# sideprotocol/plonky2-gpu

Hardware: AMD Instinct MI355X
Metric: NTTs/sec at 2^20 Goldilocks (higher is better)
Workload: dtype u64 (Goldilocks, integer modular)

## Files before the change

plonky2_gpu_amd/csrc/poseidon.h:

```cpp
#pragma once
#include "poseidon_vector.h"

namespace poseidon {

using poseidon_vector::HALF_FULL;
using poseidon_vector::N_PARTIAL;
using poseidon_vector::W;

typedef int v4i32 __attribute__((ext_vector_type(4)));
typedef int v16i32 __attribute__((ext_vector_type(16)));

#ifdef POSEIDON_MDS_NATURAL
#include POSEIDON_MDS_NATURAL
#else
struct MdsOperands {
    v4i32 A;
    v16i32 C;
};

__device__ __forceinline__ uint32_t mds_row_word(uint32_t o) {
    constexpr uint32_t WORDS[12] = POSEIDON_MDS_ROW_WORDS;
    uint32_t x = 0;
#pragma unroll
    for (int k = 0; k < 12; k++) x = o == (uint32_t)k ? WORDS[k] : x;
    return x;
}

__device__ __forceinline__ MdsOperands mds_operands() {
    const uint32_t lane = __builtin_amdgcn_mbcnt_hi(~0u, __builtin_amdgcn_mbcnt_lo(~0u, 0u));
    const uint32_t m = lane & 31, h = lane >> 5;
    const uint32_t r = (m & 3) + 4 * (m >> 3);
    const bool on = ((m >> 2) & 1) == h && r < 12;
    MdsOperands o;
#pragma unroll
    for (int w = 0; w < 3; w++) o.A[w] = on ? (int)mds_row_word((4 * w + 12 - r) % 12) : 0;
    o.A[3] = 0;
#pragma unroll
    for (int k = 0; k < 16; k++) o.C[k] = POSEIDON_MDS_PLANE_OFFSET;
    asm volatile("" : "+v"(o.A), "+v"(o.C));
    return o;
}

__device__ __forceinline__ void require_full_wave() {
    if (__builtin_amdgcn_read_exec() != ~0ull) __builtin_trap();
}

#ifdef POSEIDON_MDS_LAYER
#include POSEIDON_MDS_LAYER
#else
__device__ __forceinline__ void mds_layer(uint64_t (&s)[W], const MdsOperands &ops, const uint32_t *__restrict__ xy) {
    v4i32 T[8];
#pragma unroll
    for (int G = 0; G < 3; G++)
#pragma unroll
        for (int h = 0; h < 2; h++) {
            const uint32_t r0 = (uint32_t)(s[4 * G] >> (32 * h)), r1 = (uint32_t)(s[4 * G + 1] >> (32 * h));
            const uint32_t r2 = (uint32_t)(s[4 * G + 2] >> (32 * h)), r3 = (uint32_t)(s[4 * G + 3] >> (32 * h));
            const uint32_t a01 = __builtin_amdgcn_perm(r1, r0, 0x05010400u), c01 = __builtin_amdgcn_perm(r1, r0, 0x07030602u);
            const uint32_t a23 = __builtin_amdgcn_perm(r3, r2, 0x05010400u), c23 = __builtin_amdgcn_perm(r3, r2, 0x07030602u);
            T[4 * h + 0][G] = (int)(__builtin_amdgcn_perm(a23, a01, 0x05040100u) ^ 0x80808080u);
            T[4 * h + 1][G] = (int)(__builtin_amdgcn_perm(a23, a01, 0x07060302u) ^ 0x80808080u);
            T[4 * h + 2][G] = (int)(__builtin_amdgcn_perm(c23, c01, 0x05040100u) ^ 0x80808080u);
            T[4 * h + 3][G] = (int)(__builtin_amdgcn_perm(c23, c01, 0x07060302u) ^ 0x80808080u);
        }
    const uint32_t x0l = (uint32_t)s[0], x0h = (uint32_t)(s[0] >> 32);
    uint64_t al[W], ah[W];
    {
        const v16i32 D0 = __builtin_amdgcn_mfma_i32_32x32x32_i8(ops.A, T[0], ops.C, 0, 0, 0), D2 = __builtin_amdgcn_mfma_i32_32x32x32_i8(ops.A, T[2], ops.C, 0, 0, 0);
        const v16i32 D1 = __builtin_amdgcn_mfma_i32_32x32x32_i8(ops.A, T[1], ops.C, 0, 0, 0), D3 = __builtin_amdgcn_mfma_i32_32x32x32_i8(ops.A, T[3], ops.C, 0, 0, 0);
#pragma unroll
        for (int r = 0; r < W; r++) {
            const uint32_t Al = (uint32_t)D0[r] | ((uint32_t)D2[r] << 16), Bl = (uint32_t)D1[r] | ((uint32_t)D3[r] << 16);
            al[r] = ((uint64_t)xy[2 * r] << 32) | Al;
            asm("v_mad_u64_u32 %0, vcc, %1, %2, %0" : "+v"(al[r]) : "v"(Bl), "s"(256u) : "vcc");
        }
    }
    {
        const v16i32 D4 = __builtin_amdgcn_mfma_i32_32x32x32_i8(ops.A, T[4], ops.C, 0, 0, 0), D6 = __builtin_amdgcn_mfma_i32_32x32x32_i8(ops.A, T[6], ops.C, 0, 0, 0);
        const v16i32 D5 = __builtin_amdgcn_mfma_i32_32x32x32_i8(ops.A, T[5], ops.C, 0, 0, 0), D7 = __builtin_amdgcn_mfma_i32_32x32x32_i8(ops.A, T[7], ops.C, 0, 0, 0);
#pragma unroll
        for (int r = 0; r < W; r++) {
            const uint32_t Ah = (uint32_t)D4[r] | ((uint32_t)D6[r] << 16), Bh = (uint32_t)D5[r] | ((uint32_t)D7[r] << 16);
            ah[r] = ((uint64_t)xy[2 * r + 1] << 32) | Ah;
            asm("v_mad_u64_u32 %0, vcc, %1, %2, %0" : "+v"(ah[r]) : "v"(Bh), "s"(256u) : "vcc");
        }
    }
    asm("v_mad_u64_u32 %0, vcc, %2, %4, %0\n\t"
        "v_mad_u64_u32 %1, vcc, %3, %4, %1"
        : "+v"(al[0]), "+v"(ah[0])
        : "v"(x0l), "v"(x0h), "n"(POSEIDON_MDS_DIAG0)
        : "vcc");
#pragma unroll
    for (int r = 0; r < W; r++) s[r] = gl::fold96(al[r], ah[r]);
}

#endif
#endif

__device__ __forceinline__ void full_round(uint64_t (&s)[W], const MdsOperands &ops, const uint32_t *__restrict__ xy) {
#pragma unroll
    for (int i = 0; i < W; i++) s[i] = gl::pow7(s[i]);
    mds_layer(s, ops, xy);
}

__device__ __forceinline__ void permute(uint64_t (&s)[W], const MdsOperands &ops) {
    require_full_wave();
#pragma unroll
    for (int i = 0; i < W; i++) s[i] = gl::add_canonical(s[i], POSEIDON_ALL_ROUND_CONSTANTS[i]);
#pragma unroll 1
    for (int r = 0; r < HALF_FULL; r++) full_round(s, ops, POSEIDON_MDS_XY + 2 * W * r);
#pragma unroll 1
    for (int r = HALF_FULL; r < HALF_FULL + N_PARTIAL; r++) {
        s[0] = gl::pow7(s[0]);
        mds_layer(s, ops, POSEIDON_MDS_XY + 2 * W * r);
    }
#pragma unroll 1
    for (int r = HALF_FULL + N_PARTIAL; r < 2 * HALF_FULL + N_PARTIAL; r++) full_round(s, ops, POSEIDON_MDS_XY + 2 * W * r);
}

}
```

plonky2_gpu_amd/csrc/poseidon_limb_constants.h:

```cpp
#pragma once
#include <stdint.h>
#ifndef POSEIDON_CONST
#define POSEIDON_CONST static const
#endif
#define POSEIDON_PARTIAL_BLOCK_TERMS 297

POSEIDON_CONST uint64_t POSEIDON_INIT_STREAM_C0[121] __attribute__((aligned(64))) = {
    0x80772dc2645b280bULL, 0xe796d293a47a64cbULL, 0xdcedab70f40718baULL, 0xf4a437f2888ae909ULL,
    0xf97abba0dffb6c50ULL, 0x7f8e41e0b0a6cdffULL, 0x726af914971c1374ULL, 0x64dd936da878404dULL,
    0x85418a9fef8a9890ULL, 0x156048ee7a738154ULL, 0xd841e8ef9dde8ba0ULL, 0xdc927721da922cf8ULL,
    0xb124c33152a2421aULL, 0x14a4a64da0b2668fULL, 0xc537d44dc2875403ULL, 0x5e40f0c9bb82aab5ULL,
    0x4b1ba8d40afca97dULL, 0x1d7f8a2cce1a9d00ULL, 0x4db9a2ead2bd7262ULL, 0xd8a2eb7ef5e707adULL,
    0x91f7562377e81df5ULL, 0x156048ee7a738154ULL, 0xc1978156516879adULL, 0x0ee5dc0ce131268aULL,
    0x4715b8e5ab34653bULL, 0x7f68007619fd8ba9ULL, 0x5996a80497e24a6bULL, 0x623708f28fca70e8ULL,
    0x18737784700c75cdULL, 0xbe2e19f6d07f1a83ULL, 0xbfe85ababed2d882ULL, 0xd8a2eb7ef5e707adULL,
    0x85418a9fef8a9890ULL, 0x90e80c591f48b603ULL, 0xa9032a52f930fae6ULL, 0x1e8916a99c93a88eULL,
    0xa4911db6a32612daULL, 0x07084430a7307c9aULL, 0xbf150dc4914d380fULL, 0x7fb45d605dd82838ULL,
    0x02290fe23c20351aULL, 0xbe2e19f6d07f1a83ULL, 0x4db9a2ead2bd7262ULL, 0x64dd936da878404dULL,
    0x3a2432625475e3aeULL, 0x7e33ca8c814280deULL, 0xbba4b5d86b9a3b2cULL, 0x2f7e9aade3fdaec1ULL,
    0xad2f570a5b8545aaULL, 0xc26a083554767106ULL, 0x862361aeab0f9b6eULL, 0x7fb45d605dd82838ULL,
    0x18737784700c75cdULL, 0x1d7f8a2cce1a9d00ULL, 0x726af914971c1374ULL, 0x00a2d4321cca94feULL,
    0xad11180f69a8c29eULL, 0xe76649f9bd5d5c2eULL, 0xe7ffd578da4ea43dULL, 0xab7f81fef4274770ULL,
    0x753b8b1126665c22ULL, 0xc26a083554767106ULL, 0xbf150dc4914d380fULL, 0x623708f28fca70e8ULL,
    0x4b1ba8d40afca97dULL, 0x7f8e41e0b0a6cdffULL, 0x77736f524010c932ULL, 0xc75ac6d5b5a10ff3ULL,
// ... 478 lines not shown
    0x4cdb240000000000ULL, 0x004e640000000000ULL, 0xc0539dd594c2eb25ULL, 0x53a4361a08c316b6ULL,
    0xb8899f8b277ef3a5ULL, 0xdd56375f98e8540aULL, 0x20d61b073e4d24ccULL, 0x0eaa137ccdfcaeedULL,
    0x4bd5386cb93533f0ULL, 0xa92f07522603d627ULL, 0x79442e109481d1b7ULL, 0x90bb65609b16866aULL,
    0x14ac4d5b709acc24ULL, 0x6188d0c1cbd8533eULL, 0xb110adc5ffc6f63aULL, 0x50ae6232ffffc1cdULL,
    0x9f6aa442ffffffbdULL, 0x4cdb240000000000ULL, 0x004e640000000000ULL, 0xc8c9a691f64cf04aULL,
    0x4ee06eac4803f9d2ULL, 0xef75547931cea75cULL, 0x509c4977f0df603dULL, 0x6bcad519b6a4680dULL,
    0x96ac65b9ee5f7156ULL, 0xfe3d76217a264e25ULL, 0x27e0c04ae42f912dULL, 0x76c119b2058a2a42ULL,
    0xbfc4898b7337bacfULL, 0x7d6abe160558056aULL, 0xce2601ac466ca224ULL, 0x6188d0c1cbd8533eULL,
    0xb110adc5ffc6f63aULL, 0x50ae6232ffffc1cdULL, 0x9f6aa442ffffffbdULL, 0x4cdb240000000000ULL,
    0x004e640000000000ULL, 0x4fbdff13b945cae5ULL, 0x36077a68e217ddc4ULL, 0xa16b9056ee536ff4ULL,
    0x6f90ce44d6523d8fULL, 0x4545ea2780307b14ULL, 0xde188deac917d1a0ULL, 0x2f6cd10ea2c7415aULL,
    0x0032d62b81ce4f49ULL, 0x68e53b0c643d5a60ULL, 0x1f565def76440b0eULL, 0xcd963151269f4c14ULL,
    0xaee48b63151f6cf1ULL, 0xce2601ac466ca224ULL, 0x6188d0c1cbd8533eULL, 0xb110adc5ffc6f63aULL,
    0x50ae6232ffffc1cdULL, 0x9f6aa442ffffffbdULL, 0x4cdb240000000000ULL, 0x004e640000000000ULL,
    0xc3e553c640e2f627ULL, 0x6129993ec2f23203ULL, 0xc8c12f675f4a311fULL, 0x2e9055ab3feb7226ULL,
    0xaa2f94298328fa67ULL, 0x3aa2cd0e195d72d5ULL, 0xeb96c11d2ba82d97ULL, 0xd2eaf60942c686c8ULL,
    0x0a0781d3857dbb7aULL, 0x4bff0687c17fb73cULL, 0x20829e1121be8986ULL, 0x09eff43fc38db9cdULL,
    0xaee48b63151f6cf1ULL, 0xce2601ac466ca224ULL, 0x6188d0c1cbd8533eULL, 0xb110adc5ffc6f63aULL,
    0x50ae6232ffffc1cdULL, 0x9f6aa442ffffffbdULL, 0x4cdb240000000000ULL, 0x004e640000000000ULL,
    0x82124bbd051fc758ULL, 0x182c413a98d88851ULL, 0x703aca58966b498aULL, 0x5d40546d4259451cULL,
    0x85efc9ddc2389549ULL, 0x683141d10a2580ecULL, 0x7f14503670bb9c01ULL, 0x3423c537de869e0aULL,
    0x11dfc42b97c160faULL, 0xe2b5aa9a9ed4d540ULL, 0x180bfc04feba6fccULL, 0x93e511ff2f214401ULL,
    0x09eff43fc38db9cdULL, 0xaee48b63151f6cf1ULL, 0xce2601ac466ca224ULL, 0x6188d0c1cbd8533eULL,
    0xb110adc5ffc6f63aULL, 0x50ae6232ffffc1cdULL, 0x9f6aa442ffffffbdULL, 0x4cdb240000000000ULL,
    0x004e640000000000ULL, 0x3c72d754b84cea98ULL, 0x72fd1e97d56494daULL, 0xfdd528147a800c90ULL,
    0x69f4ae409e14b190ULL, 0x31bbb09fcc35af60ULL, 0x6ba3f325ffc76cdaULL, 0x5ef29dc4ffffc23bULL,
    0x4c5ce043ffffffbcULL, 0x47dc600000000000ULL, 0x004c000000000000ULL, 0x0000500000000000ULL,
    0xf6754bac41d188f1ULL, 0xc9e9e8c22168e4f9ULL, 0x06eb78e061df7f6eULL, 0xda550f299e7a10abULL,
    0x5721ef3cd09930c3ULL, 0xb562ee26ffcc31d9ULL, 0x1b6558bfffffc740ULL, 0x5b56203cffffffc3ULL,
    0x42db200000000000ULL, 0x005d400000000000ULL, 0x0000880000000000ULL, 0x4ea6bd499ea511e9ULL,
    0x9e5bc61b931f9ec5ULL, 0xc167f24a3b9a79c7ULL, 0x7b4e75e7fd4b21e8ULL, 0x3c63baa9cb88dd56ULL,
    0xfddef831ffc69fceULL, 0x6047d698ffffc167ULL, 0x143e1843ffffffbcULL, 0x4d2a580000000000ULL,
    0x0045380000000000ULL, 0x0000480000000000ULL, 0xcb5c52d5a439fe0dULL, 0xbf73379506c3ebe5ULL,
    0xa340b60b8b47de82ULL, 0xdd379ecee40e9d06ULL, 0x3d720756d0e1b4a9ULL, 0x5fb4b57effcc8681ULL,
    0x49f8f433ffffc7ccULL, 0x123d3c3dffffffc2ULL, 0x433dfc0000000000ULL, 0x004c7c0000000000ULL,
    0x00009c0000000000ULL, 0xea231a946ac6c26aULL, 0x8fb9fe055fac72cfULL, 0x61a2e9179c4336ceULL,
    0x64286e4accdd5d85ULL, 0xce3ccec7cb547d38ULL, 0x01405989ffc67276ULL, 0x2ff98b05ffffc0faULL,
    0x549f4c43ffffffbcULL, 0x49340c0000000000ULL, 0x0059ec0000000000ULL, 0x0000340000000000ULL,
    0x23bfe07c96e52509ULL, 0x675cd2dd5b461196ULL, 0x218e7dd3c14759c7ULL, 0xe31bb6c37bd4cd0cULL,
    0x4760004acafb03b5ULL, 0xa2077e05ffc605faULL, 0x0b64433fffffc0c0ULL, 0x0da68444ffffffbbULL,
    0x4fe2840000000000ULL, 0x004dc40000000000ULL, 0x0000340000000000ULL, 0xf47208ed0dd292bfULL,
    0x7c0de42d324421e4ULL, 0x08b3e1b289905464ULL, 0xe8b496ec3273c8e6ULL, 0x2d68aa33cdefb5ccULL,
    0x3ded0f9dffc95062ULL, 0x91879bb4ffffc44bULL, 0xbcbce040ffffffbfULL, 0x45f1600000000000ULL,
    0x0048c00000000000ULL, 0x0000700000000000ULL, 0xf20c883ffd83c064ULL, 0xd3633a161f2810f8ULL,
    0xe741c972500558a2ULL, 0x24bb9832d06db79bULL, 0x75daff51c92850aeULL, 0x2b513c52ffc413adULL,
    0x589d91a0ffffbe5fULL, 0x8b2a5046ffffffb9ULL, 0x4cb2500000000000ULL, 0x0060b00000000000ULL,
    0x0000080000000000ULL, 0x28b6e2a7c4612060ULL, 0xbcf8538e4c81c079ULL, 0x711cb1f50b1d6224ULL,
    0xf278288605e2174aULL, 0xeb9c1cc8cb922337ULL, 0xd12595d0ffc6aa2fULL, 0x8dbd7e7fffffc180ULL,
    0x28a7c043ffffffbcULL, 0x4d3f000000000000ULL, 0x004da00000000000ULL, 0x0000400000000000ULL,
    0x5b9d8087c5ddd8dbULL, 0x6b71eb5c31ba931dULL, 0xe799d7986ab1847eULL, 0xd5f75a6b61bea969ULL,
    0x80fcb72fd053ccd0ULL, 0x7d3f19c1ffcbea3eULL, 0xc4fbbceaffffc715ULL, 0xa7d7043dffffffc2ULL,
    0x4282440000000000ULL, 0x003cc40000000000ULL, 0x0000a40000000000ULL, 0x550810f4d60c836bULL,
    0x41065b24228d5d31ULL, 0x7f0db99480d05ea8ULL, 0x2f6f8fe32bc933edULL, 0xe08adac7cbbc6938ULL,
    0x25e4de42ffc6e5bdULL, 0x83db8290ffffc16fULL, 0xd8974442ffffffbdULL, 0x4a25840000000000ULL,
    0x0057240000000000ULL, 0x00003c0000000000ULL,
};

#define POSEIDON_MDS_ROW_WORDS {0x10290f11u, 0x0210290fu, 0x1c021029u, 0x0d1c0210u, 0x0d0d1c02u, 0x270d0d1cu, 0x12270d0du, 0x2212270du, 0x14221227u, 0x11142212u, 0x0f111422u, 0x290f1114u}
#define POSEIDON_MDS_PLANE_OFFSET 32768
#define POSEIDON_MDS_DIAG0 8

POSEIDON_CONST uint32_t POSEIDON_MDS_XY[720] __attribute__((aligned(64))) = {
    0x7d4b40a3u, 0x08dd377fu, 0x9b8ea8e0u, 0xbe3e71aau, 0x0d16df22u, 0xb6a23a8cu, 0x93eecc47u, 0x1095f87fu,
    0x0cdfd3f0u, 0x23abe934u, 0xfd7b015eu, 0x70cf3f63u, 0xa7be7ab2u, 0xf2707305u, 0x91a93619u, 0x51b790c8u,
    0x958db98bu, 0x4039b805u, 0xdc62ad13u, 0xe6fc00f4u, 0x1b38723eu, 0x6963b419u, 0xc922e83au, 0xf7344452u,
    0x0bd863cdu, 0xde21ff7eu, 0x8b09cd56u, 0x6a659ff3u, 0xfe10254eu, 0xf9c6ee9au, 0xb51970dbu, 0xcd7da250u,
    0x9073326bu, 0x1cf4d376u, 0xa94a2d54u, 0x0307aca2u, 0x68ed8564u, 0xe73d5278u, 0x68ac854eu, 0xeef4cfbeu,
    0xd39cb892u, 0x931f1a7cu, 0x6640103eu, 0xa7629bb1u, 0xcb7634b1u, 0x24eaf29fu, 0x127b826eu, 0x163d69cdu,
    0x10d2eafau, 0x81d46bedu, 0x6fd0a772u, 0x01169a7au, 0xb1204affu, 0x507d13e3u, 0xe1b5922au, 0x8db99cadu,
    0x64d56371u, 0x181eb35fu, 0xe883b5b5u, 0x795b9bc6u, 0x97b3c511u, 0xee28848au, 0x0556a27cu, 0x463ef8cdu,
    0x90c27cb5u, 0x57fbc1a9u, 0xdc9b42b7u, 0x19257967u, 0x4aa0a17fu, 0xf6108b40u, 0x7161df70u, 0x34d529cfu,
    0x5511ec9bu, 0xe7b20bf7u, 0x8606cf7du, 0xa840ce44u, 0x156d214eu, 0x59dcbcbau, 0xff74753au, 0x21c87284u,
    0xb8521bb8u, 0xa2b2157cu, 0xa6231c1au, 0xfcbb295eu, 0xbb7f9e02u, 0xb5840cf7u, 0xea4e8f0fu, 0x68d86cfeu,
    0x95d0fe97u, 0x13fdb8b9u, 0xe31a9e2cu, 0x44de4e5cu, 0x1ad8586eu, 0xe212f76du, 0x416b1589u, 0xb95be98bu,
    0x97bf27d2u, 0xd9728273u, 0x28b41300u, 0x6a9cf061u, 0x5d15c720u, 0x503d9405u, 0xdf663a85u, 0x66c1bb41u,
    0x1d4ec3edu, 0x470e33a8u, 0x2f128705u, 0xf509e9e8u, 0x1131e668u, 0x9b86fa0fu, 0x83873129u, 0xb3b0b8b2u,
    0xcf4a5deau, 0x18a0004au, 0x5a9ea6dau, 0x36403dc6u, 0x3d728a8au, 0x943f636eu, 0xb1ab0e1eu, 0x59ba39fdu,
    0xa1c142e7u, 0xf7ebd7c4u, 0x17a146dfu, 0x2be935b3u, 0x7bf858d9u, 0x3a158ae4u, 0xb90c0427u, 0x1090a744u,
    0x10d4d292u, 0x58d11b01u, 0x7d4fe00eu, 0xe12b528eu, 0x5fd4f48eu, 0xffebb77au, 0x6c52d15du, 0xc688b135u,
    0x630f5cadu, 0xa7cf0cefu, 0x8d06b75du, 0xefbea0deu, 0x67467522u, 0x1e9929b1u, 0x54379c01u, 0x11cd434fu,
    0xc5dbe551u, 0x25a910b8u, 0x9e6ee872u, 0x3bf19fc3u, 0x0ff9efc4u, 0x7f9e0e7du, 0x4032c3e6u, 0x690c8477u,
    0xf61dbe52u, 0x70e72a9cu, 0xeceb0ac6u, 0xe1f8dee6u, 0x33c17f27u, 0x1d4b8f3fu, 0x61c27839u, 0x946fc710u,
    0x0af65bceu, 0x005a3111u, 0xd73cad47u, 0x1b04c343u, 0xf1b8b359u, 0x6f2ea8cfu, 0x9c827028u, 0x099f0d64u,
    0x3505debfu, 0x3c53ee72u, 0x338623d0u, 0x50152ac0u, 0x8fd1493bu, 0x7d6df523u, 0x6e653f66u, 0x21184458u,
    0x62163f4au, 0x15f8e2fau, 0xdf6f6e7au, 0x0c21e9ccu, 0xf8550594u, 0xd9490c79u, 0x7fced201u, 0x81a01339u,
    0x4493b9c6u, 0x86cc1b89u, 0x26b58618u, 0x8602bb61u, 0x8419603eu, 0x1808b8ceu, 0x0123723du, 0x5c45c9dfu,
    0x9fa5a65fu, 0x3d496139u, 0x17e60d77u, 0x257d84edu, 0xfe3cce7fu, 0xe4372f18u, 0x6eb18146u, 0xd2dd812au,
    0x41290130u, 0x4afcfc74u, 0xdb83adcau, 0x51373f83u, 0x2d2fc472u, 0x3229223eu, 0x86615f67u, 0xa1e4f145u,
    0x4b750e34u, 0x17e6254bu, 0x748cd80eu, 0x2b0d2b61u, 0x679a3d1bu, 0x51a3e8f2u, 0x2a85a256u, 0x86224893u,
    0x5d1c83c9u, 0x7359a8f4u, 0x47773baeu, 0xed4fb40au, 0x3ad3cbc8u, 0x05eb3eeeu, 0x330cb1d0u, 0x83a8bf2du,
    0x880aed55u, 0xd21ccbabu, 0x68786438u, 0x492d4d2eu, 0x70f49ecfu, 0x162e41deu, 0xf6e564afu, 0x81a97f04u,
    0x29f908ebu, 0xeaae1d7bu, 0x37ab1b49u, 0x610c4be7u, 0x2746bcb2u, 0x944cf1c6u, 0x8c7e3355u, 0x9c7f07afu,
    0xc3c9eb8du, 0x6cda7c78u, 0x953b5ceeu, 0x9e42631eu, 0x9d91a162u, 0x385b00e3u, 0xdc34dd40u, 0x9b2d8642u,
    0xa0d40c26u, 0x21102899u, 0x5652213du, 0xac4713ddu, 0x5ff97265u, 0x52dae480u, 0xe33bbc09u, 0x5b6315f4u,
    0xcdc36804u, 0x5baf4127u, 0x9c0601b6u, 0x841b6c21u, 0xd6448796u, 0xd7bb6139u, 0x68758d60u, 0xb3d82dbcu,
    0x98c43ee3u, 0x7cdd2ba7u, 0xb863b895u, 0x802659f6u, 0xddeed6d2u, 0x45120f04u, 0x7744fb8bu, 0xb81eaefbu,
    0x60922f52u, 0x91313d97u, 0x3f5181efu, 0xe7c68f36u, 0x5660ac01u, 0x8f235693u, 0x508d8bf1u, 0xfd0e304du,
    0x5360b322u, 0x96d50908u, 0x039d5c83u, 0x1544bec9u, 0x43f0f4bbu, 0xda4aab0bu, 0x8f4e6c60u, 0x9687d702u,
    0x1f79b1f7u, 0x3ac569bbu, 0x457a8f71u, 0x960472c8u, 0xc636e856u, 0xee2b1e03u, 0x8d3fcb15u, 0xbc827fcfu,
    0xe8be8b93u, 0xeed4fa99u, 0x1deaa0f2u, 0x8cf27015u, 0x5bec4377u, 0x684f2a98u, 0x71772164u, 0x7119035eu,
    0x94094edcu, 0xca477399u, 0xb537d9a8u, 0x5b006578u, 0xaa8d4996u, 0x8e5ba507u, 0x3942c1f1u, 0xa40e5647u,
    0xa4c4dd90u, 0xd28b2808u, 0x64926265u, 0x22193750u, 0xf0720fe1u, 0xc0ae3f7fu, 0x5f86bb54u, 0x8fdaf131u,
    0x2ee9394fu, 0xecd39fc0u, 0xa31f9015u, 0x69b24aa8u, 0xfd40cd25u, 0x1462e136u, 0x9cdb910cu, 0x5a7a2ee3u,
    0xca46d728u, 0xd9715b28u, 0xe3df9aa4u, 0x6d836c50u, 0xa7a44e24u, 0x36105e26u, 0x9b58b205u, 0xc962bbe7u,
    0x2518b58fu, 0xd4b3e034u, 0x681e696cu, 0xa0b51609u, 0x233d02bdu, 0xcb8798a5u, 0xde6973ebu, 0x12da1f50u,
    0x3aa5a3a5u, 0xaa2039deu, 0xd94090e5u, 0x0e6ce672u, 0x1ac22b57u, 0x78000635u, 0x710f7f66u, 0x028ca693u,
    0x47a4c99au, 0x0e920130u, 0x711d920du, 0x6c71fe8eu, 0xdb465f3du, 0xeaf9c0a4u, 0x7c858f89u, 0x0e53ebabu,
    0xbea7bb7fu, 0x4da17aecu, 0xf8ee56dcu, 0x0e967cf6u, 0xf4905100u, 0x5e7f657eu, 0xdcb4b173u, 0x644fe0b6u,
    0x87b9fbe1u, 0x8bdb4653u, 0x3e51cebdu, 0x5e5eeea2u, 0xc6733fb7u, 0x3c70b65eu, 0x34afe13au, 0x63ad6e11u,
    0x7528c6d2u, 0x0232d919u, 0x689174d4u, 0xc7b0f0d2u, 0xf0a965f0u, 0x688cfed3u, 0xff33212eu, 0x4fd70d31u,
    0xde229353u, 0xff3e8bbdu, 0xb802af6bu, 0x2015b030u, 0x992abebbu, 0x565c54e2u, 0xfef5f46au, 0x3cb11eccu,
    0xd3f14796u, 0xa948fdc7u, 0x96255966u, 0xcfe7d97bu, 0x7247a583u, 0xb732e0bcu, 0x383292eeu, 0x58ae1449u,
    0xa9abd0a2u, 0xaaf3b02cu, 0x3eac6ff7u, 0xd0c7429bu, 0x1239bbb3u, 0x048563c1u, 0x6d7b4671u, 0xffa413e8u,
    0xa8ef1f34u, 0x5a10683bu, 0x6adccc53u, 0x5aeea650u, 0xb1cd83acu, 0xd2a36ff1u, 0xf94b7f68u, 0x2c603489u,
    0xd75dd0f9u, 0x4c8dbbd0u, 0x9cd71dbau, 0x39b09c9cu, 0xd81d8fe9u, 0x02700ea8u, 0x13b03b25u, 0xd01ba159u,
    0x688dec4bu, 0x511add69u, 0xd1689630u, 0xef69f42cu, 0xaecec6d0u, 0x9708e5cbu, 0x5f21563eu, 0x8f9617fcu,
    0x521bab97u, 0xeaeb1d26u, 0x194d9f88u, 0x834ef899u, 0x144fc141u, 0x51204a11u, 0xcaa5d91eu, 0xc6796bf7u,
    0x37209366u, 0x43c5f13au, 0xdc1e3f6au, 0x5f950181u, 0x1c9d43eau, 0x97d159a2u, 0x31826650u, 0x5c4cbcaau,
    0xd0200682u, 0xa79da858u, 0x42a31218u, 0xaefb2df3u, 0xa7d63858u, 0x1b926af1u, 0x856bbfe5u, 0x19860d7cu,
    0xbe6cf588u, 0x2a2fe2cdu, 0xe88bfa7fu, 0x74477d5du, 0x2b9fe3d9u, 0x7c1117a0u, 0x3a16d54cu, 0x3c6d6af3u,
    0xaf912bc2u, 0xb012c4adu, 0xa9b5c2f3u, 0xe43fb7ceu, 0x4bce3792u, 0xe1e1e768u, 0xff600a87u, 0x5524635du,
    0x12fb0cbdu, 0xa76c387cu, 0x98f010bfu, 0xbb2d38a4u, 0x5defef83u, 0x8b197802u, 0xd6b25c23u, 0x09363d01u,
    0xf9e48394u, 0xf301238au, 0x351975e6u, 0x2ae019f0u, 0x9c7eda2fu, 0xe769b9eau, 0xa11354cdu, 0xb80eaf3eu,
    0x3756ba30u, 0xc226badfu, 0x08f02b9au, 0x4790a929u, 0xfea59eccu, 0xa938728fu, 0xf1e5c441u, 0x78ac7e6bu,
    0xf09cad3cu, 0x06e8c1bcu, 0x2116d89cu, 0x014f23f7u, 0x0f9a533cu, 0x084575a9u, 0x99f3c3fbu, 0xf60de247u,
    0x01b8dfd9u, 0x8e476c3bu, 0x2e610d15u, 0x8ad1aabbu, 0x57b0397eu, 0x4901a604u, 0x05fccfe9u, 0x88f50d3eu,
    0xd500922fu, 0x304112cau, 0x1720d592u, 0x87403ad0u, 0x46d40973u, 0x6ca2750eu, 0x20fe847fu, 0xdf9a50f9u,
    0x8de5f895u, 0xa3eb9938u, 0xe4299c4du, 0x5ce65362u, 0xa10fb6eeu, 0x1ce93b55u, 0xf5f0542cu, 0xa89c812fu,
    0xc7b5bf54u, 0x165c6c98u, 0xdc0044fcu, 0x70ffdad9u, 0xd91ae0f9u, 0xf14b5607u, 0x541c594fu, 0xdb06e087u,
    0x35286e31u, 0x37f20ae8u, 0x13bd5223u, 0xcbdcf717u, 0xd28a4eabu, 0x1937c674u, 0xa4dd90beu, 0x5eee9aeau,
    0xbb829fbbu, 0x17bf307du, 0x9371659fu, 0xa50b5033u, 0xde32efe7u, 0xdd6f6178u, 0x783c8cbfu, 0xfa0c71b8u,
    0x9fbf07c5u, 0xada2dda5u, 0xb3cef37au, 0x725fa2c2u, 0xa70aa9ccu, 0xb2ddf13du, 0xbce8f7b1u, 0x487463a1u,
    0xb7c76e4du, 0xcaeb1066u, 0x69b86346u, 0x69483185u, 0x9c66c8b7u, 0x32f5eacbu, 0x908ba833u, 0x6e61a584u,
    0xb6ac24f3u, 0x8ac41a60u, 0x5bcd34b0u, 0x03217491u, 0xc1e1f3b8u, 0x8aeffdf9u, 0xbe658446u, 0x8bbab13fu,
    0xf038730eu, 0x24406053u, 0x40446364u, 0x2ebe78a4u, 0x024f76d1u, 0x271aa95eu, 0xc6f0967fu, 0x640cd11au,
    0x7565228cu, 0x056ab6e3u, 0x7253e67au, 0xf544d392u, 0x5b90169eu, 0xd936deddu, 0x293d9799u, 0x2df94a22u,
    0x205bcf46u, 0xffa9ade4u, 0x0e41e7adu, 0x2fa87429u, 0x942b4236u, 0x82b9cb53u, 0xe3779ad0u, 0x4648591cu,
    0xa198afffu, 0xa5c42321u, 0xdbbf9f8eu, 0x3ce48177u, 0xb1a4a47du, 0x5099cf97u, 0x272dd8e0u, 0xede69828u,
    0xbc7adeebu, 0x28290107u, 0x89b128ddu, 0x77f7a8c8u, 0xec17863eu, 0x259d4110u, 0x4f2eff54u, 0x9658ccbau,
    0x37a15cdfu, 0xe855d591u, 0x7dc1fa30u, 0xdb8c2f94u, 0x808e3087u, 0x7664ed2bu, 0x333d99afu, 0x8ced2c36u,
    0x47cd7aa2u, 0x9f348748u, 0xd9f6f044u, 0x959a0ef7u, 0x885c74f7u, 0xba18057bu, 0x0cac5197u, 0xc548b64eu,
    0x0dde2333u, 0x0ea8af33u, 0x1719fa90u, 0x227cd3e4u, 0x26b1dec0u, 0x67cddb43u, 0xbd334a46u, 0xfcdaa22bu,
    0xb4c5b9d4u, 0xe9d703a4u, 0x71d63affu, 0x6912295bu, 0x905fdbccu, 0x4e5e2c88u, 0xf1936d16u, 0xb2febcbcu,
    0x5676181cu, 0x256fa1e4u, 0x660e08dfu, 0x3dbb55d0u, 0xf70fc1edu, 0x0b20fabbu, 0x01170b85u, 0x401eb73au,
    0x59f9fd3fu, 0xbc75c38du, 0xc24af495u, 0x7517c105u, 0x71a3d19du, 0x76eeb8b0u, 0xced86a37u, 0x5b6ba11au,
    0xfe68fcafu, 0x8266007cu, 0xa1b84ff1u, 0x19e029d6u, 0xf2a2df4fu, 0x7bd9afcbu, 0x320a90a7u, 0xe4412237u,
    0x411d9521u, 0xb2a39ac5u, 0x2e515b05u, 0x12688e1eu, 0x139a7350u, 0x4184e7c0u, 0xe9ce42b9u, 0x3b34e7eeu,
    0xf603774eu, 0xb4e9bcb9u, 0x89c75ed9u, 0x063637e3u, 0xca339a48u, 0xa6c8f7a3u, 0xdf0ab26bu, 0xa06eabbfu,
    0x99baadabu, 0xab892c34u, 0xf1c2a04cu, 0xffb036f2u, 0x9c99d737u, 0x4337edc8u, 0x3c73545fu, 0x801aa704u,
    0x00000000u, 0x00000000u, 0x00000000u, 0x00000000u, 0x00000000u, 0x00000000u, 0x00000000u, 0x00000000u,
    0x00000000u, 0x00000000u, 0x00000000u, 0x00000000u, 0x00000000u, 0x00000000u, 0x00000000u, 0x00000000u,
    0x00000000u, 0x00000000u, 0x00000000u, 0x00000000u, 0x00000000u, 0x00000000u, 0x00000000u, 0x00000000u,
};
```

Baseline: 132,200.

## Fuse Poseidon partial rounds in pairs via precomputed block MFMA matrices

Replaces the 22 single partial rounds (each a full MDS MFMA pass) with 11 two-round blocks. Each block uses a precomputed 13-row combined matrix in int8 MFMA to produce both the next state and the intermediate s0 in one pass. The intermediate is raised to the 7th power and injected through a small column constant. This is meant to halve the MDS/fold work across the partial rounds, at the cost of more MFMAs per block, extra operand registers loaded from a constant table, and signed 64-bit accumulation logic that must stay exact.

```diff
diff --git a/plonky2_gpu_amd/csrc/poseidon.h b/plonky2_gpu_amd/csrc/poseidon.h
--- a/plonky2_gpu_amd/csrc/poseidon.h
+++ b/plonky2_gpu_amd/csrc/poseidon.h
@@ -48,8 +48,7 @@
 #ifdef POSEIDON_MDS_LAYER
 #include POSEIDON_MDS_LAYER
 #else
-__device__ __forceinline__ void mds_layer(uint64_t (&s)[W], const MdsOperands &ops, const uint32_t *__restrict__ xy) {
-    v4i32 T[8];
+__device__ __forceinline__ void byte_planes(const uint64_t (&s)[W], v4i32 (&T)[8]) {
 #pragma unroll
     for (int G = 0; G < 3; G++)
 #pragma unroll
@@ -63,6 +62,11 @@
             T[4 * h + 2][G] = (int)(__builtin_amdgcn_perm(c23, c01, 0x05040100u) ^ 0x80808080u);
             T[4 * h + 3][G] = (int)(__builtin_amdgcn_perm(c23, c01, 0x07060302u) ^ 0x80808080u);
         }
+}
+
+__device__ __forceinline__ void mds_layer(uint64_t (&s)[W], const MdsOperands &ops, const uint32_t *__restrict__ xy) {
+    v4i32 T[8];
+    byte_planes(s, T);
     const uint32_t x0l = (uint32_t)s[0], x0h = (uint32_t)(s[0] >> 32);
     uint64_t al[W], ah[W];
     {
@@ -94,6 +98,72 @@
     for (int r = 0; r < W; r++) s[r] = gl::fold96(al[r], ah[r]);
 }
 
+#define POSEIDON_PARTIAL_BLOCK2 1
+__device__ __forceinline__ MdsOperands with_own_offset(const MdsOperands &ops) {
+    MdsOperands f;
+    f.A = ops.A;
+#pragma unroll
+    for (int k = 0; k < 16; k++) f.C[k] = POSEIDON_MDS_PLANE_OFFSET;
+    asm volatile("" : "+v"(f.C));
+    return f;
+}
+
+struct Block2Operands {
+    v4i32 N[2];
+};
+
+__device__ __forceinline__ Block2Operands block2_operands() {
+    uint32_t lane = __builtin_amdgcn_mbcnt_hi(~0u, __builtin_amdgcn_mbcnt_lo(~0u, 0u));
+    asm volatile("" : "+v"(lane));
+    Block2Operands o;
+    o.N[0] = reinterpret_cast<const v4i32 *>(POSEIDON_BLOCK2_A)[lane];
+    o.N[1] = reinterpret_cast<const v4i32 *>(POSEIDON_BLOCK2_A)[64 + lane];
+    return o;
+}
+
+__device__ __forceinline__ void partial_block2(uint64_t (&s)[W], const Block2Operands &ops, const uint64_t *__restrict__ k) {
+    constexpr uint32_t COL0[12] = POSEIDON_BLOCK2_COL0;
+    constexpr int ROWS = W + 1;
+    s[0] = gl::pow7(s[0]);
+    __builtin_amdgcn_sched_barrier(0);
+    v4i32 T[8];
+    byte_planes(s, T);
+    const v16i32 Z = {0, 0, 0, 0, 0, 0, 0, 0, 0, 0, 0, 0, 0, 0, 0, 0};
+    int E[4][ROWS];
+#pragma unroll
+    for (int g = 0; g < 4; g++) {
+        const v16i32 Qa = g == 0 ? __builtin_amdgcn_mfma_i32_32x32x32_i8(ops.N[0], T[0], Z, 0, 0, 0)
+                                 : __builtin_amdgcn_mfma_i32_32x32x32_i8(ops.N[0], T[2 * g], __builtin_amdgcn_mfma_i32_32x32x32_i8(ops.N[1], T[2 * g - 1], Z, 0, 0, 0), 0, 0, 0);
+        const v16i32 Qb = __builtin_amdgcn_mfma_i32_32x32x32_i8(ops.N[0], T[2 * g + 1], __builtin_amdgcn_mfma_i32_32x32x32_i8(ops.N[1], T[2 * g], Z, 0, 0, 0), 0, 0, 0);
+#pragma unroll
+        for (int r = 0; r < ROWS; r++) {
+            E[g][r] = Qa[r] + (Qb[r] << 8);
+            asm volatile("" : "+v"(E[g][r]));
+        }
+        __builtin_amdgcn_sched_barrier(0);
+    }
+    const v16i32 Q8 = __builtin_amdgcn_mfma_i32_32x32x32_i8(ops.N[1], T[7], Z, 0, 0, 0);
+    uint64_t yl, yh;
+    asm("v_mad_i64_i32 %0, vcc, %1, 1, %2" : "=v"(yl) : "v"(E[0][W]), "s"(k[2 * W]) : "vcc");
+    asm("v_mad_i64_i32 %0, vcc, %1, %2, %0" : "+v"(yl) : "v"(E[1][W]), "s"(65536u) : "vcc");
+    asm("v_mad_i64_i32 %0, vcc, %1, 1, %2" : "=v"(yh) : "v"(E[2][W]), "s"(k[2 * W + 1]) : "vcc");
+    asm("v_mad_i64_i32 %0, vcc, %1, %2, %0" : "+v"(yh) : "v"(E[3][W]), "s"(65536u) : "vcc");
+    const uint64_t w = gl::pow7(gl::fold96(yl, yh));
+    const uint32_t wl = (uint32_t)w, wh = (uint32_t)(w >> 32);
+#pragma unroll
+    for (int r = 0; r < W; r++) {
+        uint64_t al, ah;
+        asm("v_mad_i64_i32 %0, vcc, %1, 1, %2" : "=v"(al) : "v"(E[0][r]), "s"(k[2 * r]) : "vcc");
+        asm("v_mad_i64_i32 %0, vcc, %1, %2, %0" : "+v"(al) : "v"(E[1][r]), "s"(65536u) : "vcc");
+        asm("v_mad_u64_u32 %0, vcc, %1, %2, %0" : "+v"(al) : "v"(wl), "n"(COL0[r]) : "vcc");
+        asm("v_mad_i64_i32 %0, vcc, %1, 1, %2" : "=v"(ah) : "v"(E[2][r]), "s"(k[2 * r + 1]) : "vcc");
+        asm("v_mad_i64_i32 %0, vcc, %1, %2, %0" : "+v"(ah) : "v"(E[3][r]), "s"(65536u) : "vcc");
+        ah = (uint64_t)((uint32_t)(ah >> 32) + (uint32_t)Q8[r]) << 32 | (uint32_t)ah;
+        asm("v_mad_u64_u32 %0, vcc, %1, %2, %0" : "+v"(ah) : "v"(wh), "n"(COL0[r]) : "vcc");
+        s[r] = gl::fold96(al, ah);
+    }
+}
+
 #endif
 #endif
 
@@ -107,6 +177,24 @@
     require_full_wave();
 #pragma unroll
     for (int i = 0; i < W; i++) s[i] = gl::add_canonical(s[i], POSEIDON_ALL_ROUND_CONSTANTS[i]);
+#ifdef POSEIDON_PARTIAL_BLOCK2
+    static_assert(POSEIDON_BLOCK2_FIRST == HALF_FULL && 2 * POSEIDON_BLOCK2_COUNT == N_PARTIAL, "the blocks cover the partial rounds");
+    {
+        const MdsOperands f = with_own_offset(ops);
+#pragma unroll 1
+        for (int r = 0; r < HALF_FULL; r++) full_round(s, f, POSEIDON_MDS_XY + 2 * W * r);
+    }
+    {
+        const Block2Operands ops2 = block2_operands();
+#pragma unroll 1
+        for (int b = 0; b < POSEIDON_BLOCK2_COUNT; b++) partial_block2(s, ops2, POSEIDON_BLOCK2_K + 2 * (W + 1) * b);
+    }
+    {
+        const MdsOperands f = with_own_offset(ops);
+#pragma unroll 1
+        for (int r = HALF_FULL + N_PARTIAL; r < 2 * HALF_FULL + N_PARTIAL; r++) full_round(s, f, POSEIDON_MDS_XY + 2 * W * r);
+    }
+#else
 #pragma unroll 1
     for (int r = 0; r < HALF_FULL; r++) full_round(s, ops, POSEIDON_MDS_XY + 2 * W * r);
 #pragma unroll 1
@@ -116,6 +204,7 @@
     }
 #pragma unroll 1
     for (int r = HALF_FULL + N_PARTIAL; r < 2 * HALF_FULL + N_PARTIAL; r++) full_round(s, ops, POSEIDON_MDS_XY + 2 * W * r);
-}
-
-}
+#endif
+}
+
+}
diff --git a/plonky2_gpu_amd/csrc/poseidon_limb_constants.h b/plonky2_gpu_amd/csrc/poseidon_limb_constants.h
--- a/plonky2_gpu_amd/csrc/poseidon_limb_constants.h
+++ b/plonky2_gpu_amd/csrc/poseidon_limb_constants.h
@@ -654,3 +654,147 @@
     0x00000000u, 0x00000000u, 0x00000000u, 0x00000000u, 0x00000000u, 0x00000000u, 0x00000000u, 0x00000000u,
     0x00000000u, 0x00000000u, 0x00000000u, 0x00000000u, 0x00000000u, 0x00000000u, 0x00000000u, 0x00000000u,
 };
+
+#define POSEIDON_BLOCK2_FIRST 4
+#define POSEIDON_BLOCK2_COUNT 11
+#define POSEIDON_BLOCK2_COL0 {25, 20, 34, 18, 39, 13, 13, 28, 2, 16, 41, 15}
+POSEIDON_CONST uint32_t POSEIDON_BLOCK2_A[512] __attribute__((aligned(64))) = {
+    0x6831c999u, 0x7b71302cu, 0x00504e1fu, 0x00000000u, 0xaa948e00u, 0x4a081e50u, 0x02d84e4cu, 0x00000000u,
+    0xa8485650u, 0x5294c0a6u, 0xd832f420u, 0x00000000u, 0x9a72844eu, 0x648ef2a4u, 0x4ef40a4eu, 0x00000000u,
+    0x00000000u, 0x00000000u, 0x00000000u, 0x00000000u, 0x00000000u, 0x00000000u, 0x00000000u, 0x00000000u,
+    0x00000000u, 0x00000000u, 0x00000000u, 0x00000000u, 0x00000000u, 0x00000000u, 0x00000000u, 0x00000000u,
+    0xe453371fu, 0x7def846cu, 0x4c204e5du, 0x00000000u, 0xc26bf37bu, 0x411f4e3au, 0x4a52647du, 0x00000000u,
+    0xb0a19571u, 0x1f11e878u, 0x08948eefu, 0x00000000u, 0xf6dcaa30u, 0x4ee88248u, 0x1ec0f284u, 0x00000000u,
+    0x00000000u, 0x00000000u, 0x00000000u, 0x00000000u, 0x00000000u, 0x00000000u, 0x00000000u, 0x00000000u,
+    0x00000000u, 0x00000000u, 0x00000000u, 0x00000000u, 0x00000000u, 0x00000000u, 0x00000000u, 0x00000000u,
+    0x38fcee2cu, 0x3a7848b2u, 0x50a6a46cu, 0x00000000u, 0x4e7c5e68u, 0xc2b0f638u, 0xaaa89ae4u, 0x00000000u,
+    0x7cbd1131u, 0x6ba1dcfcu, 0x94487253u, 0x00000000u, 0x5e1109c9u, 0xf395aaeeu, 0x8e568437u, 0x00000000u,
+    0x00000000u, 0x00000000u, 0x00000000u, 0x00000000u, 0x00000000u, 0x00000000u, 0x00000000u, 0x00000000u,
+    0x00000000u, 0x00000000u, 0x00000000u, 0x00000000u, 0x00000000u, 0x00000000u, 0x00000000u, 0x00000000u,
+    0x10290f19u, 0x0d0d1c02u, 0x14221227u, 0x00000000u, 0x00000000u, 0x00000000u, 0x00000000u, 0x00000000u,
+    0x00000000u, 0x00000000u, 0x00000000u, 0x00000000u, 0x00000000u, 0x00000000u, 0x00000000u, 0x00000000u,
+    0x00000000u, 0x00000000u, 0x00000000u, 0x00000000u, 0x00000000u, 0x00000000u, 0x00000000u, 0x00000000u,
+    0x00000000u, 0x00000000u, 0x00000000u, 0x00000000u, 0x00000000u, 0x00000000u, 0x00000000u, 0x00000000u,
+    0x00000000u, 0x00000000u, 0x00000000u, 0x00000000u, 0x00000000u, 0x00000000u, 0x00000000u, 0x00000000u,
+    0x00000000u, 0x00000000u, 0x00000000u, 0x00000000u, 0x00000000u, 0x00000000u, 0x00000000u, 0x00000000u,
+    0x6831c999u, 0x7b71302cu, 0x00504e1fu, 0x00000000u, 0xaa948e00u, 0x4a081e50u, 0x02d84e4cu, 0x00000000u,
+    0xa8485650u, 0x5294c0a6u, 0xd832f420u, 0x00000000u, 0x9a72844eu, 0x648ef2a4u, 0x4ef40a4eu, 0x00000000u,
+    0x00000000u, 0x00000000u, 0x00000000u, 0x00000000u, 0x00000000u, 0x00000000u, 0x00000000u, 0x00000000u,
+    0x00000000u, 0x00000000u, 0x00000000u, 0x00000000u, 0x00000000u, 0x00000000u, 0x00000000u, 0x00000000u,
+    0xe453371fu, 0x7def846cu, 0x4c204e5du, 0x00000000u, 0xc26bf37bu, 0x411f4e3au, 0x4a52647du, 0x00000000u,
+    0xb0a19571u, 0x1f11e878u, 0x08948eefu, 0x00000000u, 0xf6dcaa30u, 0x4ee88248u, 0x1ec0f284u, 0x00000000u,
+    0x00000000u, 0x00000000u, 0x00000000u, 0x00000000u, 0x00000000u, 0x00000000u, 0x00000000u, 0x00000000u,
+    0x00000000u, 0x00000000u, 0x00000000u, 0x00000000u, 0x00000000u, 0x00000000u, 0x00000000u, 0x00000000u,
+    0x38fcee2cu, 0x3a7848b2u, 0x50a6a46cu, 0x00000000u, 0x4e7c5e68u, 0xc2b0f638u, 0xaaa89ae4u, 0x00000000u,
+    0x7cbd1131u, 0x6ba1dcfcu, 0x94487253u, 0x00000000u, 0x5e1109c9u, 0xf395aaeeu, 0x8e568437u, 0x00000000u,
+    0x00000000u, 0x00000000u, 0x00000000u, 0x00000000u, 0x00000000u, 0x00000000u, 0x00000000u, 0x00000000u,
+    0x00000000u, 0x00000000u, 0x00000000u, 0x00000000u, 0x00000000u, 0x00000000u, 0x00000000u, 0x00000000u,
+    0x10290f19u, 0x0d0d1c02u, 0x14221227u, 0x00000000u, 0x00000000u, 0x00000000u, 0x00000000u, 0x00000000u,
+    0x00000000u, 0x00000000u, 0x00000000u, 0x00000000u, 0x00000000u, 0x00000000u, 0x00000000u, 0x00000000u,
+    0x130f1614u, 0x16131218u, 0x13171113u, 0x00000000u, 0x11141413u, 0x13131614u, 0x18101414u, 0x00000000u,
+    0x150f1217u, 0x12171112u, 0x1011150fu, 0x00000000u, 0x14111911u, 0x17141017u, 0x14151311u, 0x00000000u,
+    0x00000000u, 0x00000000u, 0x00000000u, 0x00000000u, 0x00000000u, 0x00000000u, 0x00000000u, 0x00000000u,
+    0x00000000u, 0x00000000u, 0x00000000u, 0x00000000u, 0x00000000u, 0x00000000u, 0x00000000u, 0x00000000u,
+    0x12131013u, 0x12101314u, 0x140f1112u, 0x00000000u, 0x19101516u, 0x11161314u, 0x13121712u, 0x00000000u,
+    0x12141713u, 0x16141319u, 0x13171410u, 0x00000000u, 0x14131312u, 0x13131712u, 0x16111013u, 0x00000000u,
+    0x00000000u, 0x00000000u, 0x00000000u, 0x00000000u, 0x00000000u, 0x00000000u, 0x00000000u, 0x00000000u,
+    0x00000000u, 0x00000000u, 0x00000000u, 0x00000000u, 0x00000000u, 0x00000000u, 0x00000000u, 0x00000000u,
+    0x17141418u, 0x14191216u, 0x14121714u, 0x00000000u, 0x13111713u, 0x19121417u, 0x11151412u, 0x00000000u,
+    0x1112120fu, 0x10141314u, 0x140f1113u, 0x00000000u, 0x17121116u, 0x15171314u, 0x14121910u, 0x00000000u,
+    0x00000000u, 0x00000000u, 0x00000000u, 0x00000000u, 0x00000000u, 0x00000000u, 0x00000000u, 0x00000000u,
+    0x00000000u, 0x00000000u, 0x00000000u, 0x00000000u, 0x00000000u, 0x00000000u, 0x00000000u, 0x00000000u,
+    0x00000000u, 0x00000000u, 0x00000000u, 0x00000000u, 0x00000000u, 0x00000000u, 0x00000000u, 0x00000000u,
+    0x00000000u, 0x00000000u, 0x00000000u, 0x00000000u, 0x00000000u, 0x00000000u, 0x00000000u, 0x00000000u,
+    0x00000000u, 0x00000000u, 0x00000000u, 0x00000000u, 0x00000000u, 0x00000000u, 0x00000000u, 0x00000000u,
+    0x00000000u, 0x00000000u, 0x00000000u, 0x00000000u, 0x00000000u, 0x00000000u, 0x00000000u, 0x00000000u,
+    0x00000000u, 0x00000000u, 0x00000000u, 0x00000000u, 0x00000000u, 0x00000000u, 0x00000000u, 0x00000000u,
+    0x00000000u, 0x00000000u, 0x00000000u, 0x00000000u, 0x00000000u, 0x00000000u, 0x00000000u, 0x00000000u,
+    0x130f1614u, 0x16131218u, 0x13171113u, 0x00000000u, 0x11141413u, 0x13131614u, 0x18101414u, 0x00000000u,
+    0x150f1217u, 0x12171112u, 0x1011150fu, 0x00000000u, 0x14111911u, 0x17141017u, 0x14151311u, 0x00000000u,
+    0x00000000u, 0x00000000u, 0x00000000u, 0x00000000u, 0x00000000u, 0x00000000u, 0x00000000u, 0x00000000u,
+    0x00000000u, 0x00000000u, 0x00000000u, 0x00000000u, 0x00000000u, 0x00000000u, 0x00000000u, 0x00000000u,
+    0x12131013u, 0x12101314u, 0x140f1112u, 0x00000000u, 0x19101516u, 0x11161314u, 0x13121712u, 0x00000000u,
+    0x12141713u, 0x16141319u, 0x13171410u, 0x00000000u, 0x14131312u, 0x13131712u, 0x16111013u, 0x00000000u,
+    0x00000000u, 0x00000000u, 0x00000000u, 0x00000000u, 0x00000000u, 0x00000000u, 0x00000000u, 0x00000000u,
+    0x00000000u, 0x00000000u, 0x00000000u, 0x00000000u, 0x00000000u, 0x00000000u, 0x00000000u, 0x00000000u,
+    0x17141418u, 0x14191216u, 0x14121714u, 0x00000000u, 0x13111713u, 0x19121417u, 0x11151412u, 0x00000000u,
+    0x1112120fu, 0x10141314u, 0x140f1113u, 0x00000000u, 0x17121116u, 0x15171314u, 0x14121910u, 0x00000000u,
+    0x00000000u, 0x00000000u, 0x00000000u, 0x00000000u, 0x00000000u, 0x00000000u, 0x00000000u, 0x00000000u,
+    0x00000000u, 0x00000000u, 0x00000000u, 0x00000000u, 0x00000000u, 0x00000000u, 0x00000000u, 0x00000000u,
+    0x00000000u, 0x00000000u, 0x00000000u, 0x00000000u, 0x00000000u, 0x00000000u, 0x00000000u, 0x00000000u,
+    0x00000000u, 0x00000000u, 0x00000000u, 0x00000000u, 0x00000000u, 0x00000000u, 0x00000000u, 0x00000000u,
+};
+POSEIDON_CONST uint64_t POSEIDON_BLOCK2_K[286] __attribute__((aligned(64))) = {
+    0xbf386d4f00000000ULL, 0x2a017f2800000000ULL, 0xf644d73d00000000ULL, 0x4b50345500000000ULL,
+    0xf19a407700000000ULL, 0xeec4fc1a00000000ULL, 0xfd35444700000000ULL, 0x0735a8ba00000000ULL,
+    0xf26a3b3300000000ULL, 0x0761b41b00000000ULL, 0xc0ddb4f000000000ULL, 0xe209521c00000000ULL,
+    0x7a01b10800000000ULL, 0xa167351d00000000ULL, 0x6c2d38f000000000ULL, 0x3160780700000000ULL,
+    0x42cee2da00000000ULL, 0x0638032000000000ULL, 0xf0af20d300000000ULL, 0x9d93494700000000ULL,
+    0xccabeb8900000000ULL, 0xb7c3321600000000ULL, 0x1274067e00000000ULL, 0xf443a84d00000000ULL,
+    0xa0c8305600000000ULL, 0x54edfef800000000ULL, 0x8fd1945500000000ULL, 0xe0daa10c00000000ULL,
+    0xda63049c00000000ULL, 0xecfa5f6800000000ULL, 0x450f3f3500000000ULL, 0x0a9c506900000000ULL,
+    0x873b1f6f00000000ULL, 0xe39b7b3e00000000ULL, 0xfc59c8ba00000000ULL, 0x54b3963000000000ULL,
+    0x03b5e2f200000000ULL, 0x5383fbf300000000ULL, 0x7e1368dd00000000ULL, 0xb3c1c1c400000000ULL,
+    0xc7d0091a00000000ULL, 0x0e395dd700000000ULL, 0x2991c8ad00000000ULL, 0xfd8edbb200000000ULL,
+    0xee2b584900000000ULL, 0x9fbc3b5f00000000ULL, 0x3057df1400000000ULL, 0x9e564cf200000000ULL,
+    0xedf9b96b00000000ULL, 0xa5f254f600000000ULL, 0xcee4edd600000000ULL, 0xa1248d3c00000000ULL,
+    0xbf1ce9c000000000ULL, 0xa29748e400000000ULL, 0x7d69a5ad00000000ULL, 0x74093bc900000000ULL,
+    0x10eb01ad00000000ULL, 0x7b01826300000000ULL, 0x4774f34600000000ULL, 0x0a4e488500000000ULL,
+    0x0f1f98fd00000000ULL, 0x0ee3040c00000000ULL, 0x88bb882700000000ULL, 0xc34a6b2800000000ULL,
+    0xa150b54800000000ULL, 0x8e56962800000000ULL, 0xee45128800000000ULL, 0xd9c9e81200000000ULL,
+    0x41c488c400000000ULL, 0xd4304a1500000000ULL, 0x1070e2f600000000ULL, 0x125b884300000000ULL,
+    0xdee69b8d00000000ULL, 0x9f63f5ee00000000ULL, 0xd1c274d800000000ULL, 0xc643faf500000000ULL,
+    0xa8aeaee400000000ULL, 0xb8c4ddbd00000000ULL, 0x529ff06700000000ULL, 0x6ca8b4b700000000ULL,
+    0xf9bc2cf500000000ULL, 0xa739720100000000ULL, 0xe0b7a96700000000ULL, 0x9d26ec4f00000000ULL,
+    0x65aca15500000000ULL, 0x7d66d65000000000ULL, 0x0546c0e200000000ULL, 0xe6ee2b0700000000ULL,
+    0x64805e6a00000000ULL, 0x9dadcd4b00000000ULL, 0xf3f41ed600000000ULL, 0x1e8848fa00000000ULL,
+    0xf2cb408600000000ULL, 0x3edb8ac800000000ULL, 0x8c786b8e00000000ULL, 0x0e91fa1c00000000ULL,
+    0x80e3f76e00000000ULL, 0x28e6453900000000ULL, 0xc469d54400000000ULL, 0x127c23fc00000000ULL,
+    0x4e1995f300000000ULL, 0xfac8c43b00000000ULL, 0xccd2f41200000000ULL, 0xe855f8fc00000000ULL,
+    0x2a30b27200000000ULL, 0xd4939a6f00000000ULL, 0x7c7ba8b300000000ULL, 0xe4884a8600000000ULL,
+    0xaddb868b00000000ULL, 0x4257352900000000ULL, 0x3ce646d400000000ULL, 0x152421c400000000ULL,
+    0xd9160ded00000000ULL, 0xe4b6992800000000ULL, 0xd4549dc200000000ULL, 0x925e590d00000000ULL,
+    0x3af8cd3b00000000ULL, 0xaf15e4ed00000000ULL, 0x7a404dbc00000000ULL, 0x1d70870400000000ULL,
+    0x999b2e6400000000ULL, 0x3a8dd96900000000ULL, 0xe646b09800000000ULL, 0x2b56110b00000000ULL,
+    0xa86754ef00000000ULL, 0x506d1e1100000000ULL, 0xb44b473600000000ULL, 0x5477f89000000000ULL,
+    0x2882ba7c00000000ULL, 0xb640e63f00000000ULL, 0x5db3b37f00000000ULL, 0xd3eaa77500000000ULL,
+    0x5ac757f500000000ULL, 0xe5879d9c00000000ULL, 0x6bcbc0c900000000ULL, 0x86805eed00000000ULL,
+    0x9e31bd5f00000000ULL, 0x6fa201e800000000ULL, 0x1fc82cd900000000ULL, 0x9495d2c800000000ULL,
+    0x6d4bba3300000000ULL, 0x905c205500000000ULL, 0x0fe5e6a800000000ULL, 0x1b53825500000000ULL,
+    0xa08a59d400000000ULL, 0xc0b1761a00000000ULL, 0xceffd34900000000ULL, 0x4ca688c000000000ULL,
+    0x2f154dd200000000ULL, 0xcc81814100000000ULL, 0x2378418100000000ULL, 0xddb9dbd900000000ULL,
+    0x0c25f8c300000000ULL, 0x8106a7e400000000ULL, 0x2e21be1300000000ULL, 0x502f5cb900000000ULL,
+    0xcf04fb4400000000ULL, 0x0d3fc28200000000ULL, 0x21102b5c00000000ULL, 0x4e5ea4c500000000ULL,
+    0xb124e22300000000ULL, 0x5e6137c100000000ULL, 0xa28229ee00000000ULL, 0x9442682a00000000ULL,
+    0x3e89aaff00000000ULL, 0x878552ed00000000ULL, 0x1a28f78200000000ULL, 0x07b4a10f00000000ULL,
+    0x5eebdc6100000000ULL, 0x98f1396300000000ULL, 0x697e897300000000ULL, 0x13b50ae400000000ULL,
+    0x5ed13bdf00000000ULL, 0xbfebb80600000000ULL, 0x0d3b1e6100000000ULL, 0x994c631400000000ULL,
+    0xea0526d400000000ULL, 0x9470da3000000000ULL, 0x7867c59400000000ULL, 0x90057c2000000000ULL,
+    0xe72b9bd700000000ULL, 0x7aba084200000000ULL, 0xa96ec3c500000000ULL, 0x2994595800000000ULL,
+    0x35cbfee200000000ULL, 0x061a6d3f00000000ULL, 0x5e49f58b00000000ULL, 0xd39961bc00000000ULL,
+    0x3840908200000000ULL, 0xb90a8ae700000000ULL, 0x4b21da0900000000ULL, 0x9aa0285a00000000ULL,
+    0x00f382e400000000ULL, 0x7541cac200000000ULL, 0x9910232900000000ULL, 0xa275b02500000000ULL,
+    0x1d00a9e400000000ULL, 0x20ab603500000000ULL, 0xa5d3454f00000000ULL, 0x87d17f0800000000ULL,
+    0x0e68328b00000000ULL, 0x97bbb00e00000000ULL, 0xbe3e178a00000000ULL, 0x57b2678300000000ULL,
+    0x591a89d100000000ULL, 0xa02e71b700000000ULL, 0x5b24b41b00000000ULL, 0x666699ab00000000ULL,
+    0xe4b6bbd200000000ULL, 0x3261305f00000000ULL, 0x1143b22100000000ULL, 0x1ae0688600000000ULL,
+    0x2931d56b00000000ULL, 0x6ae9730800000000ULL, 0xa774fe4900000000ULL, 0x25ecc7ba00000000ULL,
+    0xfea7ba5e00000000ULL, 0x3bdab0dc00000000ULL, 0xede6a04e00000000ULL, 0xcdd60c6100000000ULL,
+    0xc9e33f3900000000ULL, 0xabc4647800000000ULL, 0xd125d82f00000000ULL, 0xd6b567c200000000ULL,
+    0x4cd7605700000000ULL, 0xae2eb08a00000000ULL, 0x5026ae4500000000ULL, 0x171bffa700000000ULL,
+    0x4bb6156d00000000ULL, 0x8dfe6e1000000000ULL, 0x7e6dfcc900000000ULL, 0xf235587700000000ULL,
+    0x02ed8c1800000000ULL, 0x6e7ca01000000000ULL, 0xf470ad8a00000000ULL, 0xaada621e00000000ULL,
+    0xe1c81d5e00000000ULL, 0x8068750300000000ULL, 0xcb6899ea00000000ULL, 0x2210694100000000ULL,
+    0xc1c803c200000000ULL, 0xc846084000000000ULL, 0x224b078c00000000ULL, 0xc869e40600000000ULL,
+    0xcd62119a00000000ULL, 0xfc6a2cb100000000ULL, 0x19cf45c700000000ULL, 0xe997e3b000000000ULL,
+    0xa71cc70500000000ULL, 0x3e71d34a00000000ULL, 0x96e93e4d00000000ULL, 0xbddd719700000000ULL,
+    0x28960b2600000000ULL, 0x0e0636a000000000ULL, 0xd681780b00000000ULL, 0xa389e49800000000ULL,
+    0xe257e10f00000000ULL, 0x2bd97ec700000000ULL, 0xd0bec7d900000000ULL, 0x91d7e91c00000000ULL,
+    0xaf6c7e3e00000000ULL, 0x51dca5b100000000ULL, 0xd4e4eafc00000000ULL, 0x4f8446d600000000ULL,
+    0x808a81f800000000ULL, 0x2c38817200000000ULL, 0xb008b49c00000000ULL, 0xa1e4219500000000ULL,
+    0x943de64e00000000ULL, 0x568506ac00000000ULL, 0x7d70984400000000ULL, 0xab8d817000000000ULL,
+    0x9bf1d56f00000000ULL, 0x2b25454300000000ULL, 0x7068ebc400000000ULL, 0x0d77522c00000000ULL,
+    0xb2f9573900000000ULL, 0x32f45d5900000000ULL, 0x2b9bb3df00000000ULL, 0x2eec437200000000ULL,
+    0x5581de7f00000000ULL, 0x3e10ac5300000000ULL, 0x90891d2e00000000ULL, 0x8ec8809700000000ULL,
+    0xf9417b9300000000ULL, 0x9fbbdcd700000000ULL,
+};
```

New measurement: 132,200. Within noise of the previous version (-0.0%).
